# togheppi/pytorch-super-resolution-model-collection

Hardware: AMD Instinct MI355X
Metric: ESPCN x4 LR->HR images/sec (infer) (higher is better)
Workload: dtype f32 storage/accumulate; fp32-faithful products on the fp16 matrix cores: operands scaled by exact powers of two, split into two fp16 planes, 3 MFMAs per product (f16x3, ~3e-7 rms vs fp64, like fp32 MFMA); 1 GPU; c2: ESPCN x4 inference, 256x256 LR, batch 64 per GPU, fp32, random-init N(0,0.02); parallelism=replicas x1 (no collective)

## Files before the change

include/srk.h:

```cpp
#ifndef SRK_H_
#define SRK_H_

#include <stddef.h>
#include <stdint.h>

#ifdef __cplusplus
extern "C" {
#endif

#define SRK_VERSION 600

typedef enum srk_status {
  SRK_OK = 0,
  SRK_ERR_BAD_ARG = -1,
  SRK_ERR_UNSUPPORTED = -2,
  SRK_ERR_LAUNCH = -3,
  SRK_ERR_WORKSPACE = -4
} srk_status;

typedef enum srk_act {
  SRK_ACT_NONE = 0,
  SRK_ACT_RELU = 1,
  SRK_ACT_PRELU = 2,
  SRK_ACT_LRELU = 3,
// ... 88 lines not shown
                               void* stream);

size_t srk_conv2d_backward_weight_grouped_workspace_bytes(const srk_conv_desc* d, int n);
int srk_conv2d_backward_weight_grouped(const srk_conv_desc* d, int n, const float* const* x, const float* const* dy,
                                       const srk_bwd_mask* masks, float* const* dw, float* const* db, float beta,
                                       void* workspace, size_t workspace_bytes, void* stream);
int srk_wgrad_reduce_defer(int on);
int srk_wgrad_reduce_flush(void* stream);

int srk_resblock2_supported(int N, int H, int W, int C);
int srk_resblock2_forward(int N, int H, int W, int C, const float* x, const float* w1_packed_fwd, const float* b1,
                          const float* w2_packed_fwd, const float* b2, float* y_mid, float* y, int algo,
                          const float* x_amax, float* y_amax, void* stream);
int srk_resblock2_backward_data(int N, int H, int W, int C, const float* dy, const float* w2_packed_bwd,
                                const float* w1_packed_bwd, const float* y_mid, float* d_mid, float* dx, int algo,
                                void* stream);

size_t srk_espcn_pair_prepared_bytes(void);
int srk_espcn_pair_prepare(const float* w1, const float* b1, void* w1_prepared, void* stream);
int srk_espcn_pair_forward(int N, int H, int W, const float* x, const void* w1_prepared, const float* b1,
                           const float* w2_packed_fwd, const float* b2, float* y, float* x_amax, int x_amax_compute,
                           float* y_amax, int force, void* stream);
int srk_espcn_pair_scans(int reset);

int srk_pixel_shuffle_forward(const float* x, float* y, int N, int H, int W, int C, int r, void* stream);
int srk_pixel_shuffle_backward(const float* dy, float* dx, int N, int H, int W, int C, int r, void* stream);

int srk_act_forward(const float* x, float* y, size_t n, int channels, int act, float slope,
                    const float* prelu_weight, int prelu_n, void* stream);
int srk_act_backward(const float* dy, const float* saved, float* dx, size_t n, int channels, int act, float slope,
                     const float* prelu_weight, int prelu_n, float* dprelu, void* stream);
int srk_axpby(const float* a, const float* b, float* out, size_t n, float alpha, float beta, void* stream);
int srk_scale_dev(const float* x, const float* alpha_dev, float* out, size_t n, void* stream);

typedef enum srk_loss { SRK_LOSS_MSE = 0, SRK_LOSS_L1 = 1, SRK_LOSS_CHARBONNIER = 2, SRK_LOSS_BCE = 3 } srk_loss;
size_t srk_loss_workspace_bytes(void);
int srk_loss_forward_backward(int kind, const float* pred, const float* target, const int64_t* target_strides,
                              int N, int C, int H, int W, float eps, float grad_scale, float* loss, float* dpred,
                              void* workspace, void* stream);

#define SRK_DRCN_MAX_D 32
int srk_drcn_head_forward(const float* Y, const float* x, const float* w, int D, int N, int C, int H, int W,
                          float* out, void* stream);
size_t srk_drcn_workspace_bytes(int D);
int srk_drcn_head_loss(const float* Y, const float* x, const float* target, const float* w, int D, int N, int C, int H,
                       int W, const float* alpha_dev, const float* reg_dev, float grad_scale, float* out, float* dY,
// ... 136 lines not shown
```

pytorch_super_resolution_model_collection_amd/_build.py:

```python
import os
import subprocess
import sys
from concurrent.futures import ThreadPoolExecutor

HERE = os.path.dirname(os.path.abspath(__file__))
CSRC = os.path.join(HERE, "csrc")
LIB = os.path.join(HERE, "libsrk.so")
SOURCES = ["api.hip", "elementwise.hip", "loss_optim.hip", "conv_generic.hip", "conv_mfma.hip", "conv_mfma_bf16.hip", "conv_bfd.hip", "conv_tapn.hip", "conv_rown.hip", "conv_bfw.hip", "conv_bfr.hip", "conv_rowsw.hip", "conv_res2.hip", "conv_c64.hip",
           "conv_wgrad_mfma.hip", "conv_wgrad_bf16.hip", "bn_linear.hip", "resize_pil.hip", "prepost.hip", "drcn.hip", "conv_pair.hip", "color.hip", "tile.hip", "ssim.hip", "dihedral.hip"]
HEADERS = ["srk_common.h", "conv_problem.h", "conv_tile.h", "pack_items.h", "conv_bfw.h", "bf16_frag.h", "color_common.h", "ssim_common.h", os.path.join("..", "..", "include", "srk.h")]
FLAGS = ["--offload-arch=gfx950", "-O3", "-std=c++17", "-fPIC", "-mcode-object-version=5",
         "-fno-gpu-rdc", "-Wall", "-Wno-unused-function"]


def _hipcc():
    for c in (os.environ.get("HIPCC"), "/opt/rocm/bin/hipcc", "hipcc"):
        if c and (os.path.isabs(c) and os.path.exists(c) or not os.path.isabs(c)):
            return c
    return "hipcc"


def _mtime(p):
    return os.path.getmtime(p) if os.path.exists(p) else 0.0


def needs_build():
    newest = max(_mtime(os.path.join(CSRC, f)) for f in SOURCES + HEADERS)
    return _mtime(LIB) < max(newest, _mtime(__file__))


def build(force=False, verbose=True):
    if not force and not needs_build():
# ... 34 lines not shown
```

pytorch_super_resolution_model_collection_amd/_lib.py:

```python
import ctypes
import os
import re

import torch

_HERE = os.path.dirname(os.path.abspath(__file__))
LIB_PATH = os.environ.get("SRK_LIB_PATH") or os.path.join(_HERE, "libsrk.so")
HEADER_PATH = os.path.join(os.path.dirname(_HERE), "include", "srk.h")

ACT_NONE, ACT_RELU, ACT_PRELU, ACT_LRELU, ACT_TANH, ACT_SIGMOID = range(6)
ALGO_AUTO, ALGO_GENERIC, ALGO_MFMA, ALGO_DIRECT, ALGO_MFMA_BF16X3, ALGO_MFMA_BF16X6, ALGO_MFMA_F16X3 = range(7)
AMAX_FLOATS = 256
LOSS_MSE, LOSS_L1, LOSS_CHARBONNIER, LOSS_BCE = range(4)
SSIM_DOMAINS = {"float": 0, "u8": 1, "y8": 2}
ACT_BY_NAME = {None: ACT_NONE, "relu": ACT_RELU, "prelu": ACT_PRELU, "lrelu": ACT_LRELU, "tanh": ACT_TANH,
               "sigmoid": ACT_SIGMOID}

c_f = ctypes.c_void_p
c_vp = ctypes.c_void_p
c_int = ctypes.c_int
c_float = ctypes.c_float
c_size = ctypes.c_size_t


# ... 38 lines not shown
    "srk_wgrad_reduce_flush": (c_int, [c_vp]),
    "srk_pack_weights_batched": (c_int, [c_f, c_vp, c_vp, c_int, c_int, c_vp, c_int, c_vp]),
    "srk_packed_weight_bytes": (c_size, [c_int, c_int, c_int, c_int, c_int]),
    "srk_conv2d_forward": (c_int, [ctypes.POINTER(ConvDesc), c_f, c_f, c_f, ctypes.POINTER(Epilogue), c_vp]),
    "srk_conv2d_forward_ex": (c_int, [ctypes.POINTER(ConvDesc), c_f, c_f, c_f, ctypes.POINTER(Epilogue),
                                      ctypes.POINTER(ConvResult), c_vp]),
    "srk_conv2d_backward_data": (c_int, [ctypes.POINTER(ConvDesc), c_f, c_f, c_f, ctypes.POINTER(BwdMask), c_f,
                                         c_vp]),
    "srk_conv2d_backward_data_relu_supported": (c_int, [ctypes.POINTER(ConvDesc), c_f, c_f, ctypes.POINTER(BwdMask)]),
    "srk_conv2d_backward_data_relu": (c_int, [ctypes.POINTER(ConvDesc), c_f, c_f, c_f, ctypes.POINTER(BwdMask), c_f,
                                              c_vp]),
    "srk_conv2d_backward_weight_workspace_bytes": (c_size, [ctypes.POINTER(ConvDesc)]),
    "srk_conv2d_backward_weight": (c_int, [ctypes.POINTER(ConvDesc), c_f, c_f, ctypes.POINTER(BwdMask), c_f, c_f,
                                           c_float, c_vp, c_size, c_vp]),
    "srk_conv2d_backward_weight_grouped_workspace_bytes": (c_size, [ctypes.POINTER(ConvDesc), c_int]),
    "srk_conv2d_backward_weight_grouped": (c_int, [ctypes.POINTER(ConvDesc), c_int, ctypes.POINTER(c_vp),
                                                   ctypes.POINTER(c_vp), ctypes.POINTER(BwdMask), ctypes.POINTER(c_vp),
                                                   ctypes.POINTER(c_vp), c_float, c_vp, c_size, c_vp]),
    "srk_resblock2_supported": (c_int, [c_int, c_int, c_int, c_int]),
    "srk_espcn_pair_prepared_bytes": (c_size, []),
    "srk_espcn_pair_prepare": (c_int, [c_f, c_f, c_vp, c_vp]),
    "srk_espcn_pair_forward": (c_int, [c_int, c_int, c_int, c_f, c_vp, c_f, c_f, c_f, c_f, c_f, c_int, c_f, c_int, c_vp]),
    "srk_espcn_pair_scans": (c_int, [c_int]),
    "srk_resblock2_forward": (c_int, [c_int, c_int, c_int, c_int, c_f, c_f, c_f, c_f, c_f, c_f, c_f, c_int, c_f, c_f,
                                      c_vp]),
    "srk_absmax": (c_int, [c_f, c_size, c_f, c_vp]),
    "srk_conv2d_f16x3_supported": (c_int, [ctypes.POINTER(ConvDesc), ctypes.POINTER(Epilogue), c_f]),
    "srk_resblock2_backward_data": (c_int, [c_int, c_int, c_int, c_int, c_f, c_f, c_f, c_f, c_f, c_f, c_int, c_vp]),
    "srk_pixel_shuffle_forward": (c_int, [c_f, c_f, c_int, c_int, c_int, c_int, c_int, c_vp]),
    "srk_pixel_shuffle_backward": (c_int, [c_f, c_f, c_int, c_int, c_int, c_int, c_int, c_vp]),
    "srk_act_forward": (c_int, [c_f, c_f, c_size, c_int, c_int, c_float, c_f, c_int, c_vp]),
    "srk_act_backward": (c_int, [c_f, c_f, c_f, c_size, c_int, c_int, c_float, c_f, c_int, c_f, c_vp]),
    "srk_axpby": (c_int, [c_f, c_f, c_f, c_size, c_float, c_float, c_vp]),
    "srk_loss_workspace_bytes": (c_size, []),
    "srk_loss_forward_backward": (c_int, [c_int, c_f, c_f, ctypes.POINTER(ctypes.c_int64), c_int, c_int, c_int,
                                          c_int, c_float, c_float, c_f, c_f, c_vp, c_vp]),
    "srk_drcn_head_forward": (c_int, [c_f, c_f, c_f, c_int, c_int, c_int, c_int, c_int, c_f, c_vp]),
    "srk_drcn_workspace_bytes": (c_size, [c_int]),
    "srk_drcn_head_loss": (c_int, [c_f, c_f, c_f, c_f, c_int, c_int, c_int, c_int, c_int, c_f, c_f, c_float, c_f, c_f,
                                   c_f, c_f, c_f, c_float, c_vp, c_size, c_vp]),
    "srk_drcn_head_backward": (c_int, [c_f, c_f, c_f, c_int, c_int, c_int, c_int, c_int, c_f, c_f, c_float, c_vp, c_size,
                                       c_vp]),
    "srk_sumsq_workspace_bytes": (c_size, []),
    "srk_sumsq": (c_int, [c_f, c_size, c_float, c_f, c_vp, c_vp]),
    "srk_sgd_step": (c_int, [c_f, c_f, c_f, c_size, c_float, c_float, c_float, c_int, c_int, c_f, c_f, c_vp]),
    "srk_adam_step": (c_int, [c_f, c_f, c_f, c_f, c_size, c_float, c_float, c_float, c_float, c_float, c_vp, c_f,
# ... 73 lines not shown
    with open(HEADER_PATH) as f:
        text = f.read()
    text = re.sub(r"/\*.*?\*/", "", text, flags=re.S)
    return sorted(set(re.findall(r"\b(srk_[a-z0-9_]+)\s*\(", text)))


def load():
    global _lib
    if _lib is not None:
        return _lib
    if not os.path.exists(LIB_PATH):
        raise RuntimeError(
            "libsrk.so not found at %s — run `python __graft_entry__.py build` (hipcc --offload-arch=gfx950). "
            "There is no CPU/eager fallback for the hot path." % LIB_PATH)
    lib = ctypes.CDLL(LIB_PATH)
    for name, (res, args) in _PROTOTYPES.items():
        fn = getattr(lib, name)
        fn.restype = res
        fn.argtypes = args
    _lib = lib
    return lib


ERR_UNSUPPORTED = -2


def check(rc, what):
    if rc != 0:
        lib = load()
        raise RuntimeError("%s failed: %s (%s)" % (what, lib.srk_status_string(rc).decode(),
                                                   lib.srk_last_error_string().decode()))


def stream_ptr():
    return ctypes.c_void_p(torch.cuda.current_stream().cuda_stream)


def ptr(t):
    if t is None:
        return None
    return ctypes.c_void_p(t.data_ptr())


def require_cuda(*tensors):
    for t in tensors:
        if t is not None and not t.is_cuda:
# ... 10 lines not shown
```

pytorch_super_resolution_model_collection_amd/csrc/conv_bfr.hip:

```cpp
#include "conv_bfw.h"

namespace srk {

constexpr int BFR_MAXBUF = 6;
constexpr int BFR_CNT_BYTES = 128;
constexpr int BFR_PIT = 3;
constexpr int BFR_NSET = 3;
constexpr int BFR_TH = 8, BFR_TW = 16, BFR_HH = 10, BFR_HW = 18, BFR_NPIX = 180;
constexpr int BFR_NPIXP = 190;

__device__ unsigned g_bfr_timeouts = 0;

__device__ __noinline__ void bfr_fail(int lane) {
  if (lane == 0) {
    atomicAdd(&g_bfr_timeouts, 1u);
    __threadfence_system();
  }
  __builtin_trap();
}

template <int NTW, int ICC, bool F16, bool CV = false, bool OMASK = false, bool RES = false>
__global__ __launch_bounds__(512, 2) void k_conv_bfr(BfwParams B) {
  static_assert(CV || !(OMASK || RES), "the output mask and the residual come with the canvas variant");
  static_assert(!(OMASK && RES), "one tensor read per output tile");
// ... 43 lines not shown
      const int u = t / 3, v = t - u * 3;
      const int tapw = (P.wh0 + P.wdh * u) * P.KW_full + (P.ww0 + P.wdw * v);
      if constexpr (CV) {
        const int pg = w / NB, o = w - pg * NB;
        const int oc = sl * NB + o, ocb = oc / B.NBfull;
        wv[i] = *reinterpret_cast<const fv4*>(B.wq + ((size_t)(tapw * ICC + cc) * B.OCb + ocb) * (size_t)(8 * B.NBfull) + pg * B.NBfull +
                                              (oc - ocb * B.NBfull));
      } else {
        wv[i] = *reinterpret_cast<const fv4*>(B.wq + (size_t)(tapw * ICC + cc) * WSLOT + w);
      }
    });
    srk_static_for<0, NLD>([&](auto ic) {
      constexpr int i = decltype(ic)::value;
      const int e = tid + i * NTHR;
      if (e < FW) *reinterpret_cast<fv4*>(wl + e) = wv[i];
    });
  }
  if (tid < 2 * BFR_MAXBUF) cnt[tid] = 0u;
  const int nblk = gridDim.x;
  int first, count;
  {
    const int per_x = B.ntiles >> 3, rem_x = B.ntiles & 7;
    const int nb_x = CV ? ((nblk + 7 - xcd) >> 3) / B.nsl : (nblk + 7 - xcd) >> 3;
    const int tiles_x = per_x + (xcd < rem_x ? 1 : 0);
    const int start_x = xcd * per_x + (xcd < rem_x ? xcd : rem_x);
    first = start_x + bi;
    count = bi < tiles_x ? (tiles_x - bi + nb_x - 1) / nb_x : 0;
  }
  const int tstride = CV ? ((nblk + 7 - xcd) >> 3) / B.nsl : (nblk + 7 - xcd) >> 3;
  const int cvS = CV ? B.cv_sep : 1;
  const int cvH = P.PH + cvS, cvW = P.PW + cvS, cvK = CV ? B.cv_kx : 1;
  auto div_h = [&](int v) { return (int)__umulhi((unsigned)v, B.cv_mh); };
  auto div_w = [&](int v) { return (int)__umulhi((unsigned)v, B.cv_mw); };
  count = __builtin_amdgcn_readfirstlane(count);

  const int img_tiles = P.tiles_x * P.tiles_y;
  int s2n, s2y, s2x;
  int a_n, a_y, a_x, b_n, b_y, b_x;
  {
    auto split = [&](int t, int& n, int& y, int& x) {
      n = t / img_tiles;
      const int q = t - n * img_tiles;
      y = q / P.tiles_x;
      x = q - y * P.tiles_x;
      n = __builtin_amdgcn_readfirstlane(n);
      y = __builtin_amdgcn_readfirstlane(y);
      x = __builtin_amdgcn_readfirstlane(x);
    };
// ... 251 lines not shown
          for (int e = 0; e < 4; ++e) v[e] = __builtin_fmaf(act_slope, fminf(v[e], 0.f), fmaxf(v[e], 0.f));
        }
        if constexpr (OMASK) {
#pragma unroll
          for (int e = 0; e < 4; ++e) v[e] = om[nt][r][e] > 0.f ? v[e] : 0.f;
        }
        if constexpr (RES) v += om[nt][r];
        rmax = fmaxf(fmaxf(fabsf(v[0]), fabsf(v[1])), rmax);
        rmax = fmaxf(fmaxf(fabsf(v[2]), fabsf(v[3])), rmax);
        pend[nt][r] = v;
      }
      if (want_amax) amax = pok ? fmaxf(amax, rmax) : amax;
    }
  };
  auto park = [&](int n, int r0, int c0) {
    if (act_kind == 1) park_kind(std::integral_constant<int, 1>{}, n, r0, c0);
    else if (act_kind == 0) park_kind(std::integral_constant<int, 0>{}, n, r0, c0);
    else park_kind(std::integral_constant<int, 2>{}, n, r0, c0);
  };
#pragma unroll
  for (int nt = 0; nt < NTW; ++nt) asm volatile("" ::"v"(bias4[nt]));
  asm volatile("" ::"v"(act_slope));
  __syncthreads();

  int o_n = grp ? b_n : a_n, o_y = grp ? b_y : a_y, o_x = grp ? b_x : a_x;
  int b = grp;
  unsigned k = 0;
  uint4 fa[3][2][NTW];
  uint4 fb[3][2];
  const uint4* hb = hal0 + (size_t)b * HBUF + lane_b;
  auto ldA = [&](auto uc, auto vc, auto ccc) {
    constexpr int u = decltype(uc)::value, v = decltype(vc)::value, cc = decltype(ccc)::value;
    const uint4* wb = wl + lane_a;
#pragma unroll
    for (int nt = 0; nt < NTW; ++nt) {
      fa[u][0][nt] = wb[((u * 3 + v) * ICC + cc) * WSLOT + nt * 16];
      fa[u][1][nt] = wb[((u * 3 + v) * ICC + cc) * WSLOT + PLANE_A + nt * 16];
    }
  };
  auto ldB = [&](const uint4* base, auto sc) {
    constexpr int s = decltype(sc)::value, v = s / 6, R = s - 6 * v;
    fb[s % 3][0] = base[R * HW + v];
    fb[s % 3][1] = base[R * HW + v + PLANE_B];
  };
  auto mfma3 = [&](auto uc, auto sc) {
    constexpr int u = decltype(uc)::value, s = decltype(sc)::value, R = s % 6, r = R - u;
// ... 67 lines not shown
            }
            __builtin_amdgcn_sched_barrier(0);
          }
          if constexpr (u == u_lo) {
            if constexpr (R == 0) {
              ldA(I2{}, std::integral_constant<int, v>{}, ccc);
              __builtin_amdgcn_sched_barrier(0);
            } else if constexpr (R >= 4) {
              if constexpr (v < 2) ldA(std::integral_constant<int, R - 4>{}, std::integral_constant<int, v + 1>{}, ccc);
              else ldA(std::integral_constant<int, R - 4>{}, I0{}, std::integral_constant<int, ccn>{});
              __builtin_amdgcn_sched_barrier(0);
            }
          }
        });
      });
      b = nb;
      k = nk;
      hb = hbn;
    });
    park(n, r0, c0);
    adv2(o_n, o_y, o_x);
  }
  srk_static_for<0, NST>([&](auto qc) { store_slot(qc); });
  if (P.ep.y_amax) amax_commit(P.ep.y_amax, amax, blockIdx.x + wave, amax_peek(P.ep.y_amax, blockIdx.x + wave));
  if (dead) bfr_fail(lane);
}

static int bfr_launch_cv(const BfwParams& B, size_t lds, int grid, hipStream_t s) {
  note_amax_written(B.P.ep.y_amax != nullptr);
  const dim3 blk(512);
  const bool omask = B.P.ep.out_relu != nullptr, res = B.P.ep.residual != nullptr;
  auto go = [&](auto f16c, auto omc, auto resc) {
    constexpr bool F = decltype(f16c)::value, O = decltype(omc)::value, R = decltype(resc)::value;
    note_kernel("k_conv_bfr<2,2%s,canvas%s%s%s>", F ? ",f16" : "", B.cv_sep ? "" : "0", O ? ",relu" : "", R ? ",res" : "");
    launch_lds<&k_conv_bfr<2, 2, F, true, O, R>>(dim3(grid), blk, lds, s, B);
  };
  if (B.w_descale && res) go(std::true_type{}, std::false_type{}, std::true_type{});
  else if (B.w_descale) go(std::true_type{}, std::false_type{}, std::false_type{});
  else if (res) go(std::false_type{}, std::false_type{}, std::true_type{});
  else if (omask) go(std::false_type{}, std::true_type{}, std::false_type{});
  else go(std::false_type{}, std::false_type{}, std::false_type{});
  return check_launch("conv_bfr");
}

template <int NTW, int ICC>
static int bfr_launch_t(const BfwParams& B, size_t lds, int grid, hipStream_t s) {
// ... 95 lines not shown
  P.tiles_x = (P.PW + BFR_TW - 1) / BFR_TW;
  const long ntiles = (long)P.tiles_x * P.tiles_y * P.N;
  if (ntiles >= (1L << 29)) return -1;
  if (mode != 1) {
    if ((double)P.PH * P.PW < 0.9 * (double)P.tiles_y * P.tiles_x * (BFR_TH * BFR_TW)) return -1;
    if (ntiles < 4L * kNumCU) return -1;
  }
  const size_t wbytes = (size_t)9 * B.ICc * 8 * B.NB * 16;
  const size_t slot_bytes = (size_t)8 * BFR_NPIXP * 16;
  const long lds_cap = 160L * 1024 - 512 - BFR_CNT_BYTES;
  long nbuf = (lds_cap - (long)wbytes) / (long)slot_bytes;
  const int want = env_int("SRK_BFR_NBUF", 0);
  if (want >= 3 && want < nbuf) nbuf = want;
  if (nbuf > BFR_MAXBUF) nbuf = BFR_MAXBUF;
  if (nbuf < 3) return -1;
  B.nbuf = (int)nbuf;
  B.NPIXp = BFR_NPIXP;
  B.late = 2;
  const size_t lds = wbytes + (size_t)nbuf * slot_bytes + BFR_CNT_BYTES;
  B.ntiles = (int)ntiles;
  B.out_bytes = (unsigned)((size_t)P.N * P.OH * P.OW * P.OC * sizeof(float));
  int grid = kNumCU;
  if (grid > ntiles) grid = (int)ntiles;
  if (ntw == 2) return B.ICc == 1 ? bfr_launch_t<2, 1>(B, lds, grid, s) : bfr_launch_t<2, 2>(B, lds, grid, s);
  return bfr_launch_t<3, 1>(B, lds, grid, s);
}

}

namespace srk {
int pair_ring_timeouts(int reset);
}
extern "C" int srk_ring_timeouts(int reset) {
  const int vp = srk::pair_ring_timeouts(reset);
  if (vp < 0) return -1;
  unsigned v = (unsigned)vp;
  unsigned vr = 0;
  if (hipMemcpyFromSymbol(&vr, HIP_SYMBOL(srk::g_bfr_timeouts), sizeof(vr)) != hipSuccess) {
    (void)hipGetLastError();
    return -1;
  }
  if (reset && vr) {
    const unsigned z = 0;
    (void)hipMemcpyToSymbol(HIP_SYMBOL(srk::g_bfr_timeouts), &z, sizeof(z));
  }
  return (int)(v + vr);
// ... 2 lines not shown
```

pytorch_super_resolution_model_collection_amd/csrc/conv_bfw.h:

```cpp
#pragma once
#include "srk_common.h"
#include "conv_problem.h"
#include "conv_tile.h"
#include "bf16_frag.h"
#include <stdlib.h>
#include <type_traits>

namespace srk {

typedef __attribute__((address_space(3))) unsigned lds_cnt_t;
constexpr unsigned kLdsCntSpinCap = 1u << 18;

__device__ __forceinline__ unsigned lds_cnt_peek(lds_cnt_t* p) {
  return (unsigned)__builtin_amdgcn_readfirstlane((int)__hip_atomic_load(p, __ATOMIC_RELAXED, __HIP_MEMORY_SCOPE_WORKGROUP));
}
__device__ __forceinline__ void lds_cnt_wait(lds_cnt_t* p, unsigned target, bool& dead) {
  if (!dead) {
    unsigned spins = 0;
    while ((int)(lds_cnt_peek(p) - target) < 0) {
      __builtin_amdgcn_s_sleep(1);
      if (++spins > kLdsCntSpinCap) {
        dead = true;
        break;
      }
// ... 2 lines not shown
  asm volatile("" ::: "memory");
}
__device__ __forceinline__ void lds_cnt_signal(lds_cnt_t* p, unsigned n = 1u) {
  asm volatile("" ::: "memory");
  if ((threadIdx.x & 63) == 0) __hip_atomic_fetch_add(p, n, __ATOMIC_RELAXED, __HIP_MEMORY_SCOPE_WORKGROUP);
  asm volatile("" ::: "memory");
}

constexpr int BFW_MAXTAPS = 32;
constexpr int BFW_IT = 6;

struct BfwParams {
  MfmaConvParams P;
  const uint4* wq;
  int ICc, NB, NPIXp, ntiles;
  const float* w_descale;
  int nsl, NBfull, OCb;
  int late;
  unsigned out_bytes;
  int nbuf;
  int cv_kx;
  int cv_sep;
  unsigned cv_mh, cv_mw;
};

static inline int bfw_group_stride(int npix) {
  const int a = npix + ((2 - npix) & 15), b = npix + ((14 - npix) & 15);
  return a < b ? a : b;
}

static bool bfw_pick_tile(int maxpix, int PH, int PW, int KHv, int KWv, long cap_px, TilePick& best) {
  bool found = false;
  long best_tiles = 0, best_halo = 0;
  const int maxTW = PW < maxpix ? PW : maxpix;
  for (int TW = 1; TW <= (maxTW > 1 ? maxTW : 1); ++TW) {
    int TH = maxpix / TW;
    if (TH > PH) TH = PH;
    for (; TH >= 1; --TH) {
      const int HH = TH - 1 + KHv, HWd = TW - 1 + KWv;
      if (bfw_group_stride(HH * HWd) > cap_px) continue;
      const long tiles = (long)cdiv(PH, TH) * cdiv(PW, TW);
      const long halo = (long)HH * HWd * tiles;
      const bool fewer = tiles < best_tiles, same = tiles == best_tiles;
      const bool wider = same && halo * 100 <= best_halo * 106 && TW > best.TW;
      const bool smaller = same && halo < best_halo && TW >= best.TW;
      if (!found || fewer || wider || smaller) {
// ... 24 lines not shown
```

pytorch_super_resolution_model_collection_amd/csrc/conv_pair.hip:

```cpp
#include "conv_bfw.h"

namespace srk {

namespace {

constexpr int PR_TH = 8, PR_TW = 16, PR_HW = 18;
constexpr int PR_NSLOTPIX = 6 * PR_HW, PR_NPIXP = PR_NSLOTPIX + 2;
constexpr int PR_NKEEP = 2 * PR_HW, PR_KP = PR_NKEEP + 2;
constexpr int PR_XR = 14, PR_XC = 23, PR_XP = 24;
constexpr int PR_NSLOT = 3, PR_NKBUF = 3;
constexpr int PR_WL2 = 9 * 2 * 256;
constexpr int PR_HBUF = 4 * PR_NPIXP;
constexpr int PR_KBUF = 2 * 4 * PR_KP;
constexpr int PR_PLANE = PR_NSLOT * PR_HBUF + PR_NKBUF * PR_KBUF;
constexpr int PR_XPQ = PR_XR * PR_XP * 16;
constexpr int PR_XT = PR_XPQ + 32;
constexpr int PR_XBUF = PR_XT + PR_XR * PR_XP * 8;
constexpr unsigned long long PR_FPIX = 0xfdb9eca875316420ull;
constexpr unsigned PR_AMAX_CAP = 1u << 14;
constexpr int PR_ARRIVE = 1, PR_DEPART = 2;
constexpr int PR_XLD = 24;
constexpr int PR_W1P = 2 * 2 * 8 * 64;
constexpr int PR_W1P_FLOATS = 144;
constexpr size_t PR_W1P_BYTES = (size_t)PR_W1P * 16 + PR_W1P_FLOATS * 4;
constexpr size_t PR_LDS = (size_t)PR_WL2 * 16 + (size_t)2 * PR_PLANE * 16 + (size_t)2 * PR_XBUF + 64;
static_assert(PR_LDS <= 160 * 1024, "k_espcn_pair: LDS");

__device__ unsigned g_pair_timeouts = 0;
__device__ unsigned g_pair_scans = 0;

typedef unsigned v4u_t __attribute__((ext_vector_type(4)));

struct PairParams {
  const float* x;
  const uint4* w1p;
  const float* b1;
  const uint4* wq2;
  const float* w2_descale;
  const float* b2;
  float* y;
  float* x_amax;
  float* y_amax;
  size_t xn;
  int amax_mode;
  int N, H, W, OH, OW, tiles_y, img_tiles, ntiles;
  unsigned x_img_bytes, y_bytes;
};

__device__ __forceinline__ float pr_slice_absmax(const float* __restrict__ x, size_t lo, size_t hi, size_t n, bool tail,
                                                 int t, int nt) {
  const f32x4* x4 = reinterpret_cast<const f32x4*>(x);
  float m = 0.f;
  for (size_t base = lo; base < hi; base += (size_t)nt * PR_XLD) {
    f32x4 v[PR_XLD];
#pragma unroll
    for (int k = 0; k < PR_XLD; ++k) {
      const size_t e = base + (size_t)t + (size_t)k * nt;
      v[k] = x4[e < hi ? e : hi - 1];
    }
#pragma unroll
    for (int k = 0; k < PR_XLD; ++k) m = abs_max4(m, v[k]);
  }
  if (tail) {
    const size_t e = (n & ~(size_t)3) + (size_t)t;
    if (t < 3 && e < n) m = fmaxf(m, fabsf(x[e]));
  }
  return m;
}

// ... 120 lines not shown
  int kmul[2], kadd[2], kd[2];
#pragma unroll
  for (int s = 0; s < 2; ++s) {
    const PrKGroup own = pr_kgroup(6 + s, kq), g = own.kind == PR_KNONE ? pr_kgroup(6 + s, kq - 1) : own;
    kmul[s] = g.kind == PR_KTAP ? 16 : 8;
    kd[s] = g.kind == PR_KTAP ? 8 : 32;
    asm volatile("" : "+v"(kd[s]));
    kadd[s] = g.kind == PR_KTAP ? 16 * (g.dy * PR_XP + g.dx - kq) : PR_XT + 8 * (g.dy * PR_XP - kq);
  }
  const int wr_slot = (kq >> 1) * PR_NPIXP * 16 + (kq & 1) * 8, wr_keep = (c1 * 4 + (kq >> 1)) * PR_KP * 16 + (kq & 1) * 8;

  const int rh = gw >> 1, nf2 = gw & 1;
  const int pj = j < 4 ? 2 * j : (j < 12 ? 2 * j - 7 : 2 * j - 16);
  const int lane_b = (4 * rh - 2) * PR_HW + pj + kq * PR_NPIXP;
  const int lane_k = pj + kq * PR_KP;
  const int lane_a = kq * 32 + nf2 * 16 + j;
  float b2v[4];
#pragma unroll
  for (int e = 0; e < 4; ++e) b2v[e] = B.b2[nf2 * 16 + 4 * kq + e];

  const int xcd = blockIdx.x & 7;
  int first, count;
  {
    const int lb = xcd * (nblk >> 3) + (xcd < (nblk & 7) ? xcd : (nblk & 7)) + (blockIdx.x >> 3);
    const int per = B.ntiles / nblk, rem = B.ntiles - per * nblk;
    first = lb * per + (lb < rem ? lb : rem);
    count = per + (lb < rem ? 1 : 0);
  }
  count = __builtin_amdgcn_readfirstlane(count);

  const __amdgpu_buffer_rsrc_t yr = buffer_rsrc(B.y, B.y_bytes);
  const unsigned HW_ = (unsigned)(B.H * B.W);
  float xv[2][3];
  auto xload = [&](int i) {
    const bool valid = i < count;
    const int t = first + (valid ? i : 0);
    const int n = t / B.img_tiles, rem = t - n * B.img_tiles;
    const int tx = rem / B.tiles_y, ty = rem - tx * B.tiles_y;
    const __amdgpu_buffer_rsrc_t xr = buffer_rsrc(B.x + (size_t)n * 3 * HW_, B.x_img_bytes);
#pragma unroll
    for (int s = 0; s < 2; ++s) {
      const int q = lt + 256 * s, qy = q / PR_XC, qx = q - qy * PR_XC;
      const bool ok = valid && q < PR_XR * PR_XC;
      const unsigned o = ok ? 4u * (unsigned)((ty * PR_TH + qy) * B.W + tx * PR_TW + qx) : 0x80000000u;
#pragma unroll
      for (int c = 0; c < 3; ++c)
        xv[s][c] = __builtin_bit_cast(float, __builtin_amdgcn_raw_buffer_load_b32(xr, (int)(o + (ok ? 4u * c * HW_ : 0u)), 0, 0));
    }
  };
  auto l1_frags = [&](auto nm, const int* off, f32x4 (*a)[2]) {
// ... 52 lines not shown
    xmax = __uint_as_float(lds_cnt_peek(cnt + 14));
    if (lds_cnt_peek(cnt + 15)) {
      float* red = reinterpret_cast<float*>(xin_all);
      const float m = wave_max(pr_slice_absmax(B.x, 0, B.xn >> 2, B.xn, true, tid, 512));
      if (lane == 0) red[wave] = m;
      __syncthreads();
#pragma unroll
      for (int i = 0; i < 8; ++i) xmax = fmaxf(xmax, red[i]);
      xmax = __uint_as_float((unsigned)__builtin_amdgcn_readfirstlane((int)__float_as_uint(xmax)));
      __syncthreads();
      if (tid == 0) atomicAdd(&g_pair_scans, 1u);
    }
  }
  for (int i = tid; i < 2 * PR_XBUF / 16; i += 512) reinterpret_cast<uint4*>(xin_all)[i] = make_uint4(0u, 0u, 0u, 0u);
  __syncthreads();
  const int kx = amax_scale_exp(xmax);
  const float bnd = wave_max(fabsf(babs) + wsum * xmax);
  const int kw1 = amax_scale_exp(w1t[128]);
  const int km = amax_scale_exp(bnd);
  const float sx1 = exp2i(kx), sxm = exp2i(km);
  const float dsc1 = exp2i(-kx) * exp2i(-kw1);
  const float dsc2 = exp2i(-km) * B.w2_descale[0];

  unsigned own = 0;
  unsigned kseq = 0;
  int typrev = 0;
  for (int i = grp; i < count; i += 2, ++own) {
    const int t = first + i;
    const int n = t / B.img_tiles, rem = t - n * B.img_tiles;
    const int tx = rem / B.tiles_y, ty = rem - tx * B.tiles_y;
    const bool fresh = i == 0 || ty == 0;
    const bool hand = i + 1 < count && ty + 1 < B.tiles_y;
    kseq = i == grp ? (grp == 0 ? 1u : 2u + (ty == 0 ? 1u : 0u))
                    : kseq + 2u + (typrev + 1 == B.tiles_y ? 1u : 0u) + (ty == 0 ? 1u : 0u);
    typrev = ty;
    const unsigned kb = kseq % PR_NKBUF, ku = kseq / PR_NKBUF, tb = (kseq - 1u) % PR_NKBUF, tu = (kseq - 1u) / PR_NKBUF;
#pragma unroll
    for (int s = 0; s < 2; ++s) {
      const int q = lt + 256 * s;
      if (q < PR_XR * PR_XC) {
        const int qy = q / PR_XC, qx = q - qy * PR_XC;
        unsigned h01, m01, h2, m2;
        split2h(xv[s][0], xv[s][1], sx1, h01, m01);
        split2h(xv[s][2], 0.f, sx1, h2, m2);
        *reinterpret_cast<uint4*>(xin + 16 * (qy * PR_XP + qx)) = make_uint4(h01, h2 | (m01 << 16), (m01 >> 16) | (m2 << 16), h01);
        unsigned short* tq = reinterpret_cast<unsigned short*>(xin + PR_XT) + 4 * (qy * PR_XP + qx);
// ... 107 lines not shown
                acc[r] = mfma16h(fa[u][0], xh, acc[r]);
              }
            }
          }
        }
        lds_cnt_signal(cnt + 3 + slot);
      }
      lds_cnt_signal(cnt + 11 + tb, fresh ? 2u : 1u);
      lds_cnt_signal(cnt + 11 + kb, hand ? 1u : 2u);
      const int oc = tx * PR_TW + pj;
#pragma unroll
      for (int r = 0; r < 4; ++r) {
        const int orow = ty * PR_TH + 4 * rh + r;
        const bool ok = oc < B.OW && orow < B.OH;
        f32x4 v;
#pragma unroll
        for (int e = 0; e < 4; ++e) v[e] = fmaxf(__builtin_fmaf(acc[r][e], dsc2, b2v[e]), 0.f);
        if (ok) amax = fmaxf(amax, fmaxf(fmaxf(v[0], v[1]), fmaxf(v[2], v[3])));
        const unsigned o = ok ? 4u * (unsigned)(((n * B.OH + orow) * B.OW + oc) * 32 + nf2 * 16 + 4 * kq) : 0x80000000u;
        __builtin_amdgcn_raw_buffer_store_b128(__builtin_bit_cast(v4u_t, v), yr, (int)o, 0, 0);
      }
    }
  }
  if (B.y_amax) amax_commit(B.y_amax, amax, blockIdx.x + wave, amax_peek(B.y_amax, blockIdx.x + wave));
  if (dead && lane == 0) atomicAdd(&g_pair_timeouts, 1u);
}

}

int espcn_pair_launch(int N, int H, int W, const float* x, const void* w1p, const float* b1, const void* wp2,
                      const float* b2, float* y, float* x_amax, int amax_mode, float* y_amax, bool force, hipStream_t s) {
  if (N < 1 || H < 7 || W < 7 || !x_amax) return -1;
  const int OH = H - 6, OW = W - 6;
  const int tiles_y = (OH + PR_TH - 1) / PR_TH, tiles_x = (OW + PR_TW - 1) / PR_TW;
  const long ntiles = (long)N * tiles_y * tiles_x;
  const size_t x_img = (size_t)3 * H * W * 4, y_bytes = (size_t)N * OH * OW * 32 * 4;
  if (ntiles >= (1L << 29) || x_img >= (1ull << 31) || y_bytes >= (1ull << 31)) return -1;
  if (!force) {
    if ((double)OH * OW < 0.85 * (double)tiles_y * tiles_x * (PR_TH * PR_TW)) return -1;
    if (ntiles < 4L * kNumCU) return -1;
  }
  const size_t elems = (size_t)9 * 64 * 32;
  const char* prepared = reinterpret_cast<const char*>(wp2) + bf3_prepared_offset(elems);
  const char* fsec = prepared + f16_section_offset(64, 32, 9);
  PairParams B{};
  B.x = x; B.w1p = reinterpret_cast<const uint4*>(w1p); B.b1 = b1; B.b2 = b2; B.y = y; B.x_amax = x_amax; B.y_amax = y_amax;
  B.xn = (size_t)N * 3 * H * W;
  B.amax_mode = amax_mode;
  B.wq2 = reinterpret_cast<const uint4*>(fsec);
  B.w2_descale = reinterpret_cast<const float*>(fsec + bf3_main_bytes(64, 32, 9));
  B.N = N; B.H = H; B.W = W; B.OH = OH; B.OW = OW; B.tiles_y = tiles_y; B.img_tiles = tiles_x * tiles_y;
  B.ntiles = (int)ntiles;
  B.x_img_bytes = (unsigned)x_img;
  B.y_bytes = (unsigned)y_bytes;
  int grid = kNumCU;
  if (grid > ntiles) grid = (int)ntiles;
  note_amax_written(y_amax != nullptr);
  note_kernel("k_espcn_pair");
  launch_lds<&k_espcn_pair>(dim3(grid), dim3(512), PR_LDS, s, B);
  return check_launch("espcn_pair");
}

int pair_ring_timeouts(int reset) {
  unsigned v = 0;
  if (hipMemcpyFromSymbol(&v, HIP_SYMBOL(g_pair_timeouts), sizeof(v)) != hipSuccess) {
    (void)hipGetLastError();
    return -1;
  }
  if (reset && v) {
    const unsigned z = 0;
    (void)hipMemcpyToSymbol(HIP_SYMBOL(g_pair_timeouts), &z, sizeof(z));
  }
  return (int)v;
}

int pair_scans(int reset) {
  unsigned v = 0;
  if (hipMemcpyFromSymbol(&v, HIP_SYMBOL(g_pair_scans), sizeof(v)) != hipSuccess) {
    (void)hipGetLastError();
// ... 38 lines not shown
```

pytorch_super_resolution_model_collection_amd/csrc/srk_common.h:

```cpp
#pragma once
#include <hip/hip_runtime.h>
#include <stdint.h>
#include <stdio.h>
#include <stdarg.h>
#include <atomic>
#include <type_traits>
#include "../../include/srk.h"

namespace srk {

void set_error(const char* fmt, ...);
void note_kernel(const char* fmt, ...);
void note_amax_written(bool written);
void note_bn_partial_rows(int rows);

const char* env_str(const char* name);
int env_int(const char* name, int dflt);

inline int check_launch(const char* what) {
  hipError_t e = hipGetLastError();
  if (e != hipSuccess) {
    set_error("%s: launch failed: %s", what, hipGetErrorString(e));
    return SRK_ERR_LAUNCH;
  }
// ... 46 lines not shown
  }
};

template <auto K, typename... A>
inline void launch_lds(dim3 grid, dim3 block, size_t lds, hipStream_t s, A... args) {
  static LdsLimit lim;
  lim.ensure(reinterpret_cast<const void*>(K), lds);
  hipLaunchKernelGGL(K, grid, block, lds, s, args...);
}

inline unsigned cdiv(size_t a, size_t b) { return (unsigned)((a + b - 1) / b); }

struct Strides4 {
  int64_t n, c, h, w;
};
inline Strides4 strides4(const int64_t* s) { return {s[0], s[1], s[2], s[3]}; }

__device__ __forceinline__ int xcd_tile_index(int bx, int nb) {
  const int per = nb >> 3, rem = nb & 7;
  const int xcd = bx & 7, idx = bx >> 3;
  return xcd < rem ? xcd * (per + 1) + idx : rem * (per + 1) + (xcd - rem) * per + idx;
}

template <int I0, int I1, typename F>
__device__ __forceinline__ void srk_static_for(F&& f) {
  if constexpr (I0 < I1) {
    f(std::integral_constant<int, I0>{});
    srk_static_for<I0 + 1, I1>(f);
  }
}

__device__ __forceinline__ __amdgpu_buffer_rsrc_t buffer_rsrc(const void* base, unsigned bytes) {
  const unsigned long long a = reinterpret_cast<unsigned long long>(base);
  const unsigned lo = __builtin_amdgcn_readfirstlane((unsigned)a), hi = __builtin_amdgcn_readfirstlane((unsigned)(a >> 32));
  void* p = reinterpret_cast<void*>(((unsigned long long)hi << 32) | lo);
  return __builtin_amdgcn_make_buffer_rsrc(p, (short)0, (int)__builtin_amdgcn_readfirstlane(bytes), 0x00020000);
}

__device__ __forceinline__ f32x4 mfma16(float a, float b, f32x4 c) {
  return __builtin_amdgcn_mfma_f32_16x16x4f32(a, b, c, 0, 0, 0);
}

__device__ __forceinline__ float act_apply(float v, int act, float a) {
  switch (act) {
    case SRK_ACT_RELU: return v > 0.f ? v : 0.f;
    case SRK_ACT_PRELU:
// ... 38 lines not shown
```

Measured before the change: 73870 images/s.

## Add measured per-XCD tile split with wall-clock stamps for ESPCN pair and bfr kernels

Adds host-side machinery that splits the persistent kernels' tiles across the eight XCDs according to per-XCD throughput rates. Rates are measured by having one block per XCD write wall-clock stamps into pinned host memory and are smoothed with an EMA. The ESPCN pair kernel and the bfr conv now read per-XCD start and count from the launch struct instead of computing an equal split. The default mode is equal shares, so by default only the stamping overhead and a host mutex plus capture check are added per launch. The aim is to cut tail imbalance when some XCDs run slower.

```diff
diff --git a/include/srk.h b/include/srk.h
--- a/include/srk.h
+++ b/include/srk.h
@@ -134,6 +134,12 @@
                            const float* w2_packed_fwd, const float* b2, float* y, float* x_amax, int x_amax_compute,
                            float* y_amax, int force, void* stream);
 int srk_espcn_pair_scans(int reset);
+
+int srk_xcd_balance_mode(int mode);
+int srk_xcd_balance_force(const int permille[8]);
+int srk_xcd_balance_state(float rates[8], int last_tiles[8], unsigned long long last_ticks[8]);
+int srk_xcd_split(int ntiles, int grid, const float rates[8], int clamp, int start[8], int tiles[8]);
+int srk_xcd_split_strided(int ntiles, int grid, const float rates[8], int clamp, int start[8], int tiles[8]);
 
 int srk_pixel_shuffle_forward(const float* x, float* y, int N, int H, int W, int C, int r, void* stream);
 int srk_pixel_shuffle_backward(const float* dy, float* dx, int N, int H, int W, int C, int r, void* stream);
diff --git a/pytorch_super_resolution_model_collection_amd/_build.py b/pytorch_super_resolution_model_collection_amd/_build.py
--- a/pytorch_super_resolution_model_collection_amd/_build.py
+++ b/pytorch_super_resolution_model_collection_amd/_build.py
@@ -7,7 +7,7 @@
 CSRC = os.path.join(HERE, "csrc")
 LIB = os.path.join(HERE, "libsrk.so")
 SOURCES = ["api.hip", "elementwise.hip", "loss_optim.hip", "conv_generic.hip", "conv_mfma.hip", "conv_mfma_bf16.hip", "conv_bfd.hip", "conv_tapn.hip", "conv_rown.hip", "conv_bfw.hip", "conv_bfr.hip", "conv_rowsw.hip", "conv_res2.hip", "conv_c64.hip",
-           "conv_wgrad_mfma.hip", "conv_wgrad_bf16.hip", "bn_linear.hip", "resize_pil.hip", "prepost.hip", "drcn.hip", "conv_pair.hip", "color.hip", "tile.hip", "ssim.hip", "dihedral.hip"]
+           "conv_wgrad_mfma.hip", "conv_wgrad_bf16.hip", "bn_linear.hip", "resize_pil.hip", "prepost.hip", "drcn.hip", "conv_pair.hip", "color.hip", "tile.hip", "ssim.hip", "dihedral.hip", "xcd_balance.hip"]
 HEADERS = ["srk_common.h", "conv_problem.h", "conv_tile.h", "pack_items.h", "conv_bfw.h", "bf16_frag.h", "color_common.h", "ssim_common.h", os.path.join("..", "..", "include", "srk.h")]
 FLAGS = ["--offload-arch=gfx950", "-O3", "-std=c++17", "-fPIC", "-mcode-object-version=5",
          "-fno-gpu-rdc", "-Wall", "-Wno-unused-function"]
diff --git a/pytorch_super_resolution_model_collection_amd/_lib.py b/pytorch_super_resolution_model_collection_amd/_lib.py
--- a/pytorch_super_resolution_model_collection_amd/_lib.py
+++ b/pytorch_super_resolution_model_collection_amd/_lib.py
@@ -84,6 +84,12 @@
     "srk_espcn_pair_prepare": (c_int, [c_f, c_f, c_vp, c_vp]),
     "srk_espcn_pair_forward": (c_int, [c_int, c_int, c_int, c_f, c_vp, c_f, c_f, c_f, c_f, c_f, c_int, c_f, c_int, c_vp]),
     "srk_espcn_pair_scans": (c_int, [c_int]),
+    "srk_xcd_balance_mode": (c_int, [c_int]),
+    "srk_xcd_balance_force": (c_int, [ctypes.POINTER(c_int)]),
+    "srk_xcd_balance_state": (c_int, [ctypes.POINTER(c_float), ctypes.POINTER(c_int), ctypes.POINTER(ctypes.c_ulonglong)]),
+    "srk_xcd_split": (c_int, [c_int, c_int, ctypes.POINTER(c_float), c_int, ctypes.POINTER(c_int), ctypes.POINTER(c_int)]),
+    "srk_xcd_split_strided": (c_int, [c_int, c_int, ctypes.POINTER(c_float), c_int, ctypes.POINTER(c_int),
+                                      ctypes.POINTER(c_int)]),
     "srk_resblock2_forward": (c_int, [c_int, c_int, c_int, c_int, c_f, c_f, c_f, c_f, c_f, c_f, c_f, c_int, c_f, c_f,
                                       c_vp]),
     "srk_absmax": (c_int, [c_f, c_size, c_f, c_vp]),
@@ -203,6 +209,38 @@
     return lib
 
 
+XCD_EQUAL, XCD_MEASURED, XCD_FORCED = range(3)
+
+
+def xcd_balance_mode(mode):
+    was = load().srk_xcd_balance_mode(int(mode))
+    if was < 0:
+        check(was, "srk_xcd_balance_mode")
+    return was
+
+
+def xcd_balance_force(permille):
+    check(load().srk_xcd_balance_force((c_int * 8)(*[int(v) for v in permille])), "srk_xcd_balance_force")
+
+
+def xcd_balance_state():
+    r, t, k = (c_float * 8)(), (c_int * 8)(), (ctypes.c_ulonglong * 8)()
+    sets = load().srk_xcd_balance_state(r, t, k)
+    if sets < 0:
+        check(sets, "srk_xcd_balance_state")
+    return list(r), list(t), list(k), sets
+
+
+def xcd_split(ntiles, grid, rates, clamp=True, strided=False):
+    lib = load()
+    s, t = (c_int * 8)(), (c_int * 8)()
+    fn = lib.srk_xcd_split_strided if strided else lib.srk_xcd_split
+    rc = fn(int(ntiles), int(grid), (c_float * 8)(*[float(v) for v in rates]), int(bool(clamp)), s, t)
+    if rc < 0:
+        check(rc, "srk_xcd_split")
+    return list(s), list(t), bool(rc)
+
+
 ERR_UNSUPPORTED = -2
 
 
diff --git a/pytorch_super_resolution_model_collection_amd/csrc/conv_bfr.hip b/pytorch_super_resolution_model_collection_amd/csrc/conv_bfr.hip
--- a/pytorch_super_resolution_model_collection_amd/csrc/conv_bfr.hip
+++ b/pytorch_super_resolution_model_collection_amd/csrc/conv_bfr.hip
@@ -89,8 +89,8 @@
   {
     const int per_x = B.ntiles >> 3, rem_x = B.ntiles & 7;
     const int nb_x = CV ? ((nblk + 7 - xcd) >> 3) / B.nsl : (nblk + 7 - xcd) >> 3;
-    const int tiles_x = per_x + (xcd < rem_x ? 1 : 0);
-    const int start_x = xcd * per_x + (xcd < rem_x ? xcd : rem_x);
+    const int tiles_x = CV ? per_x + (xcd < rem_x ? 1 : 0) : B.xs.tiles[xcd];
+    const int start_x = CV ? xcd * per_x + (xcd < rem_x ? xcd : rem_x) : B.xs.start[xcd];
     first = start_x + bi;
     count = bi < tiles_x ? (tiles_x - bi + nb_x - 1) / nb_x : 0;
   }
@@ -388,6 +388,9 @@
   for (int nt = 0; nt < NTW; ++nt) asm volatile("" ::"v"(bias4[nt]));
   asm volatile("" ::"v"(act_slope));
   __syncthreads();
+  const bool stamp = !CV && __builtin_amdgcn_readfirstlane(blockIdx.x < 8 && wave == 0 && count > 0 && B.stamps != nullptr);
+  unsigned long long stamp_t0 = 0;
+  if (stamp) stamp_t0 = wall_clock64();
 
   int o_n = grp ? b_n : a_n, o_y = grp ? b_y : a_y, o_x = grp ? b_x : a_x;
   int b = grp;
@@ -501,6 +504,7 @@
     adv2(o_n, o_y, o_x);
   }
   srk_static_for<0, NST>([&](auto qc) { store_slot(qc); });
+  if (stamp) xcd_stamp(B.stamps, B.seq, stamp_t0, count);
   if (P.ep.y_amax) amax_commit(P.ep.y_amax, amax, blockIdx.x + wave, amax_peek(P.ep.y_amax, blockIdx.x + wave));
   if (dead) bfr_fail(lane);
 }
@@ -642,6 +646,12 @@
   B.out_bytes = (unsigned)((size_t)P.N * P.OH * P.OW * P.OC * sizeof(float));
   int grid = kNumCU;
   if (grid > ntiles) grid = (int)ntiles;
+  {
+    const XcdLaunch xl = xcd_balance_launch(XCD_STRIDED, B.ntiles, grid, s);
+    B.xs = xl.split;
+    B.stamps = xl.stamps;
+    B.seq = xl.seq;
+  }
   if (ntw == 2) return B.ICc == 1 ? bfr_launch_t<2, 1>(B, lds, grid, s) : bfr_launch_t<2, 2>(B, lds, grid, s);
   return bfr_launch_t<3, 1>(B, lds, grid, s);
 }
diff --git a/pytorch_super_resolution_model_collection_amd/csrc/conv_bfw.h b/pytorch_super_resolution_model_collection_amd/csrc/conv_bfw.h
--- a/pytorch_super_resolution_model_collection_amd/csrc/conv_bfw.h
+++ b/pytorch_super_resolution_model_collection_amd/csrc/conv_bfw.h
@@ -48,6 +48,9 @@
   int cv_kx;
   int cv_sep;
   unsigned cv_mh, cv_mw;
+  XcdSplit xs;
+  unsigned* stamps;
+  unsigned seq;
 };
 
 static inline int bfw_group_stride(int npix) {
diff --git a/pytorch_super_resolution_model_collection_amd/csrc/conv_pair.hip b/pytorch_super_resolution_model_collection_amd/csrc/conv_pair.hip
--- a/pytorch_super_resolution_model_collection_amd/csrc/conv_pair.hip
+++ b/pytorch_super_resolution_model_collection_amd/csrc/conv_pair.hip
@@ -45,6 +45,9 @@
   int amax_mode;
   int N, H, W, OH, OW, tiles_y, img_tiles, ntiles;
   unsigned x_img_bytes, y_bytes;
+  XcdSplit xs;
+  unsigned* stamps;
+  unsigned seq;
 };
 
 __device__ __forceinline__ float pr_slice_absmax(const float* __restrict__ x, size_t lo, size_t hi, size_t n, bool tail,
@@ -211,10 +214,11 @@
   const int xcd = blockIdx.x & 7;
   int first, count;
   {
-    const int lb = xcd * (nblk >> 3) + (xcd < (nblk & 7) ? xcd : (nblk & 7)) + (blockIdx.x >> 3);
-    const int per = B.ntiles / nblk, rem = B.ntiles - per * nblk;
-    first = lb * per + (lb < rem ? lb : rem);
-    count = per + (lb < rem ? 1 : 0);
+    const int nb_x = (nblk + 7 - xcd) >> 3, k = blockIdx.x >> 3;
+    const int tiles_x = B.xs.tiles[xcd];
+    const int per = tiles_x / nb_x, rem = tiles_x - per * nb_x;
+    first = B.xs.start[xcd] + k * per + (k < rem ? k : rem);
+    count = per + (k < rem ? 1 : 0);
   }
   count = __builtin_amdgcn_readfirstlane(count);
 
@@ -313,6 +317,9 @@
   const float dsc1 = exp2i(-kx) * exp2i(-kw1);
   const float dsc2 = exp2i(-km) * B.w2_descale[0];
 
+  const bool stamp = __builtin_amdgcn_readfirstlane(blockIdx.x < 8 && wave == 0 && count > 0 && B.stamps != nullptr);
+  unsigned long long stamp_t0 = 0;
+  if (stamp) stamp_t0 = wall_clock64();
   unsigned own = 0;
   unsigned kseq = 0;
   int typrev = 0;
@@ -466,6 +473,7 @@
       }
     }
   }
+  if (stamp) xcd_stamp(B.stamps, B.seq, stamp_t0, count);
   if (B.y_amax) amax_commit(B.y_amax, amax, blockIdx.x + wave, amax_peek(B.y_amax, blockIdx.x + wave));
   if (dead && lane == 0) atomicAdd(&g_pair_timeouts, 1u);
 }
@@ -499,6 +507,12 @@
   B.y_bytes = (unsigned)y_bytes;
   int grid = kNumCU;
   if (grid > ntiles) grid = (int)ntiles;
+  {
+    const XcdLaunch xl = xcd_balance_launch(XCD_RUNS, B.ntiles, grid, s);
+    B.xs = xl.split;
+    B.stamps = xl.stamps;
+    B.seq = xl.seq;
+  }
   note_amax_written(y_amax != nullptr);
   note_kernel("k_espcn_pair");
   launch_lds<&k_espcn_pair>(dim3(grid), dim3(512), PR_LDS, s, B);
diff --git a/pytorch_super_resolution_model_collection_amd/csrc/srk_common.h b/pytorch_super_resolution_model_collection_amd/csrc/srk_common.h
--- a/pytorch_super_resolution_model_collection_amd/csrc/srk_common.h
+++ b/pytorch_super_resolution_model_collection_amd/csrc/srk_common.h
@@ -92,6 +92,30 @@
   return xcd < rem ? xcd * (per + 1) + idx : rem * (per + 1) + (xcd - rem) * per + idx;
 }
 
+struct XcdSplit {
+  int start[8];
+  int tiles[8];
+};
+enum { XCD_RUNS = 0, XCD_STRIDED = 1 };
+constexpr float kXcdClamp = 0.08f;
+constexpr int kXcdMinTilesPerBlock = 64;
+bool xcd_split(int ntiles, int grid, const float rates[8], bool clamp, int order, XcdSplit& out);
+struct XcdLaunch {
+  XcdSplit split;
+  unsigned* stamps;
+  unsigned seq;
+};
+XcdLaunch xcd_balance_launch(int order, int ntiles, int grid, hipStream_t s);
+
+__device__ __forceinline__ void xcd_stamp(unsigned* slots, unsigned seq, unsigned long long t0, int tiles) {
+  typedef unsigned xs4 __attribute__((ext_vector_type(4)));
+  const unsigned long long t1 = wall_clock64();
+  if ((threadIdx.x & 63) == 0) {
+    const xs4 v = {seq, (unsigned)(t1 - t0), (unsigned)tiles, seq};
+    *reinterpret_cast<xs4*>(slots + 4 * (blockIdx.x & 7)) = v;
+  }
+}
+
 template <int I0, int I1, typename F>
 __device__ __forceinline__ void srk_static_for(F&& f) {
   if constexpr (I0 < I1) {
diff --git a/pytorch_super_resolution_model_collection_amd/csrc/xcd_balance.hip b/pytorch_super_resolution_model_collection_amd/csrc/xcd_balance.hip
--- /dev/null
+++ b/pytorch_super_resolution_model_collection_amd/csrc/xcd_balance.hip
@@ -0,0 +1,276 @@
+#include "srk_common.h"
+#include <math.h>
+#include <mutex>
+#include <string.h>
+
+namespace srk {
+
+namespace {
+
+constexpr int kOrders = 2, kMaxDev = 64, kIssueRing = 16;
+constexpr float kEmaWeight = 0.25f;
+
+inline int xcd_blocks(int grid, int x) { return (grid + 7 - x) >> 3; }
+
+void equal_shares(int ntiles, int grid, int order, int base[8]) {
+  bool orphan = false;
+  if (order == XCD_STRIDED) {
+    for (int x = 0; x < 8; ++x) {
+      base[x] = (ntiles >> 3) + (x < (ntiles & 7) ? 1 : 0);
+      orphan = orphan || (base[x] > 0 && xcd_blocks(grid, x) == 0);
+    }
+    if (!orphan) return;
+  }
+  const int per = ntiles / grid, rem = ntiles - per * grid;
+  for (int x = 0, lb = 0; x < 8; ++x) {
+    const int nb = xcd_blocks(grid, x), extra = rem - lb < 0 ? 0 : (rem - lb > nb ? nb : rem - lb);
+    base[x] = nb * per + extra;
+    lb += nb;
+  }
+}
+
+void fill(const int share[8], XcdSplit& out) {
+  for (int x = 0, s = 0; x < 8; ++x) {
+    out.start[x] = s;
+    out.tiles[x] = share[x];
+    s += share[x];
+  }
+}
+
+}
+
+bool xcd_split(int ntiles, int grid, const float rates[8], bool clamp, int order, XcdSplit& out) {
+  int base[8];
+  if (ntiles < 0) ntiles = 0;
+  if (grid < 1) grid = 1;
+  equal_shares(ntiles, grid, order, base);
+  bool ok = rates != nullptr, same = true;
+  for (int x = 0; ok && x < 8; ++x) {
+    const float r = rates[x];
+    ok = isfinite(r) && (clamp ? r > 0.f : r >= 0.f);
+    same = same && r == rates[0];
+  }
+  double wsum = 0.0, w[8];
+  int lo[8], hi[8];
+  for (int x = 0; ok && x < 8; ++x) {
+    w[x] = (double)base[x] * (double)rates[x];
+    wsum += w[x];
+    if (clamp) {
+      lo[x] = (int)floor((double)base[x] * (1.0 - kXcdClamp));
+      hi[x] = (int)ceil((double)base[x] * (1.0 + kXcdClamp));
+    } else {
+      lo[x] = w[x] > 0.0 && ntiles >= 8 ? 1 : 0;
+      hi[x] = w[x] > 0.0 ? ntiles : 0;
+    }
+  }
+  if (!ok || !(wsum > 0.0) || !isfinite(wsum) || same) {
+    fill(base, out);
+    return ok && wsum > 0.0 && isfinite(wsum);
+  }
+  double v[8];
+  bool held[8] = {};
+  for (int round = 0; round < 8; ++round) {
+    double left = ntiles, wfree = 0.0;
+    for (int x = 0; x < 8; ++x) {
+      if (held[x]) left -= v[x];
+      else wfree += w[x];
+    }
+    int worst = -1;
+    double excess = 0.0;
+    for (int x = 0; x < 8; ++x) {
+      if (held[x]) continue;
+      v[x] = wfree > 0.0 ? w[x] * left / wfree : 0.0;
+      const double e = v[x] < lo[x] ? lo[x] - v[x] : (v[x] > hi[x] ? v[x] - hi[x] : 0.0);
+      if (e > excess) {
+        excess = e;
+        worst = x;
+      }
+    }
+    if (worst < 0) break;
+    v[worst] = v[worst] < lo[worst] ? lo[worst] : hi[worst];
+    held[worst] = true;
+  }
+  int share[8], sum = 0;
+  for (int x = 0; x < 8; ++x) {
+    share[x] = (int)floor(v[x]);
+    if (share[x] < lo[x]) share[x] = lo[x];
+    if (share[x] > hi[x]) share[x] = hi[x];
+    sum += share[x];
+  }
+  while (sum != ntiles) {
+    const int step = sum < ntiles ? 1 : -1;
+    int pick = -1;
+    double best = 0.0;
+    for (int x = 0; x < 8; ++x) {
+      if (step > 0 ? share[x] >= hi[x] : share[x] <= lo[x]) continue;
+      const double d = (v[x] - share[x]) * step;
+      if (pick < 0 || d > best) {
+        best = d;
+        pick = x;
+      }
+    }
+    if (pick < 0) {
+      fill(base, out);
+      return false;
+    }
+    share[pick] += step;
+    sum += step;
+  }
+  fill(share, out);
+  return true;
+}
+
+namespace {
+
+struct Issue {
+  unsigned seq;
+  int tiles[8];
+};
+struct DeviceState {
+  unsigned* slots = nullptr;
+  bool tried = false;
+  float rates[8] = {1.f, 1.f, 1.f, 1.f, 1.f, 1.f, 1.f, 1.f};
+  unsigned seq = 0;
+  unsigned taken[kOrders] = {};
+  int sets = 0;
+  Issue issued[kOrders][kIssueRing] = {};
+  int last_tiles[8] = {};
+  unsigned long long last_ticks[8] = {};
+};
+std::mutex g_mu;
+DeviceState g_dev[kMaxDev];
+int g_mode = 0;
+float g_force[8] = {1.f, 1.f, 1.f, 1.f, 1.f, 1.f, 1.f, 1.f};
+
+void consume(DeviceState& S, int order) {
+  if (!S.slots) return;
+  const volatile unsigned* p = S.slots + order * 32;
+  unsigned w[8][4];
+  for (int x = 0; x < 8; ++x)
+    for (int i = 0; i < 4; ++i) w[x][i] = p[4 * x + i];
+  const unsigned seq = w[0][0];
+  if (seq == 0 || (int)(seq - S.taken[order]) <= 0 || (int)(S.seq - seq) < 0) return;
+  double r[8], mean = 0.0;
+  for (int x = 0; x < 8; ++x) {
+    if (w[x][0] != seq || w[x][3] != seq || w[x][1] == 0 || w[x][2] == 0) return;
+    r[x] = (double)w[x][2] / (double)w[x][1];
+    mean += r[x] / 8.0;
+  }
+  S.taken[order] = seq;
+  const Issue& is = S.issued[order][seq % kIssueRing];
+  double m2 = 0.0;
+  for (int x = 0; x < 8; ++x) {
+    double rel = r[x] / mean;
+    rel = rel < 1.0 - kXcdClamp ? 1.0 - kXcdClamp : (rel > 1.0 + kXcdClamp ? 1.0 + kXcdClamp : rel);
+    S.rates[x] = (1.f - kEmaWeight) * S.rates[x] + kEmaWeight * (float)rel;
+    m2 += S.rates[x] / 8.0;
+    S.last_ticks[x] = w[x][1];
+    S.last_tiles[x] = is.seq == seq ? is.tiles[x] : (int)w[x][2];
+  }
+  for (int x = 0; x < 8; ++x) S.rates[x] = (float)(S.rates[x] / m2);
+  ++S.sets;
+}
+
+DeviceState* current_state() {
+  int dev = -1;
+  if (hipGetDevice(&dev) != hipSuccess || dev < 0 || dev >= kMaxDev) {
+    (void)hipGetLastError();
+    return nullptr;
+  }
+  return &g_dev[dev];
+}
+
+}
+
+XcdLaunch xcd_balance_launch(int order, int ntiles, int grid, hipStream_t s) {
+  XcdLaunch L{};
+  std::lock_guard<std::mutex> lock(g_mu);
+  DeviceState* S = current_state();
+  bool capturing = false;
+  if (s) {
+    hipStreamCaptureStatus st = hipStreamCaptureStatusNone;
+    if (hipStreamIsCapturing(s, &st) == hipSuccess) capturing = st != hipStreamCaptureStatusNone;
+    else (void)hipGetLastError();
+  }
+  const bool takes_part = S && grid >= 8 && (long)ntiles >= (long)kXcdMinTilesPerBlock * grid;
+  if (takes_part && !capturing) {
+    if (!S->tried) {
+      S->tried = true;
+      void* p = nullptr;
+      if (hipHostMalloc(&p, kOrders * 32 * sizeof(unsigned), hipHostMallocDefault) == hipSuccess && p) {
+        memset(p, 0, kOrders * 32 * sizeof(unsigned));
+        S->slots = reinterpret_cast<unsigned*>(p);
+      } else {
+        (void)hipGetLastError();
+      }
+    }
+    consume(*S, order);
+  }
+  const float ones[8] = {1.f, 1.f, 1.f, 1.f, 1.f, 1.f, 1.f, 1.f};
+  if (g_mode == 2) xcd_split(ntiles, grid, g_force, false, order, L.split);
+  else xcd_split(ntiles, grid, g_mode == 1 && takes_part ? S->rates : ones, true, order, L.split);
+  if (takes_part && !capturing && S->slots) {
+    L.stamps = S->slots + order * 32;
+    L.seq = ++S->seq;
+    if (L.seq == 0) L.seq = ++S->seq;
+    Issue& is = S->issued[order][L.seq % kIssueRing];
+    is.seq = L.seq;
+    memcpy(is.tiles, L.split.tiles, sizeof(is.tiles));
+  }
+  return L;
+}
+
+}
+
+extern "C" int srk_xcd_balance_mode(int mode) {
+  SRK_REQUIRE(mode >= 0 && mode <= 2, "xcd_balance_mode: 0 (equal), 1 (measured) or 2 (forced), got %d", mode);
+  std::lock_guard<std::mutex> lock(srk::g_mu);
+  const int was = srk::g_mode;
+  srk::g_mode = mode;
+  return was;
+}
+
+extern "C" int srk_xcd_balance_force(const int permille[8]) {
+  SRK_REQUIRE(permille, "xcd_balance_force: null pointer");
+  long sum = 0;
+  for (int x = 0; x < 8; ++x) {
+    SRK_REQUIRE(permille[x] >= 0 && permille[x] <= 1000000, "xcd_balance_force: rate %d out of range", permille[x]);
+    sum += permille[x];
+  }
+  SRK_REQUIRE(sum > 0, "xcd_balance_force: all rates are zero");
+  std::lock_guard<std::mutex> lock(srk::g_mu);
+  for (int x = 0; x < 8; ++x) srk::g_force[x] = (float)permille[x] * 1e-3f;
+  return SRK_OK;
+}
+
+extern "C" int srk_xcd_balance_state(float rates[8], int last_tiles[8], unsigned long long last_ticks[8]) {
+  std::lock_guard<std::mutex> lock(srk::g_mu);
+  srk::DeviceState* S = srk::current_state();
+  SRK_REQUIRE(S, "xcd_balance_state: no current device");
+  for (int o = 0; o < srk::kOrders; ++o) srk::consume(*S, o);
+  for (int x = 0; x < 8; ++x) {
+    if (rates) rates[x] = S->rates[x];
+    if (last_tiles) last_tiles[x] = S->last_tiles[x];
+    if (last_ticks) last_ticks[x] = S->last_ticks[x];
+  }
+  return S->sets;
+}
+
+static int split_api(int ntiles, int grid, const float rates[8], int clamp, int order, int start[8], int tiles[8]) {
+  SRK_REQUIRE(ntiles >= 0 && grid >= 1 && rates && start && tiles, "xcd_split: bad argument");
+  srk::XcdSplit sp;
+  const bool used = srk::xcd_split(ntiles, grid, rates, clamp != 0, order, sp);
+  for (int x = 0; x < 8; ++x) {
+    start[x] = sp.start[x];
+    tiles[x] = sp.tiles[x];
+  }
+  return used ? 1 : 0;
+}
+
+extern "C" int srk_xcd_split(int ntiles, int grid, const float rates[8], int clamp, int start[8], int tiles[8]) {
+  return split_api(ntiles, grid, rates, clamp, srk::XCD_RUNS, start, tiles);
+}
+
+extern "C" int srk_xcd_split_strided(int ntiles, int grid, const float rates[8], int clamp, int start[8], int tiles[8]) {
+  return split_api(ntiles, grid, rates, clamp, srk::XCD_STRIDED, start, tiles);
+}
```

Result: no change. 73840 images/s (-0.0%).
